# vklyukin/nf_distillation

Hardware: NVIDIA B200
Metric: kd_train_samples_per_sec (higher is better)
Workload: dtype bf16

## Files before the change

nf_distillation_b200/csrc/zpath.cu:

```cuda
#include <cuda_bf16.h>
#include <cuda_runtime.h>
#include <cstdint>

#include "../../include/nfk.h"
#include "launch_util.h"
#include "ptx.cuh"

namespace nfk {

constexpr int ZT = 256;

__device__ __forceinline__ uint32_t bf2(float lo, float hi) {
  __nv_bfloat162 v = __floats2bfloat162_rn(lo, hi);
  return *reinterpret_cast<uint32_t*>(&v);
}

__device__ __forceinline__ void sigmoid_logsigmoid(float t, float& s, float& ls) {
  const float e = expf(-fabsf(t));
  const float l1p = log1pf(e);
  if (t >= 0.f) {
    s = 1.f / (1.f + e);
    ls = -l1p;
  } else {
    s = e / (1.f + e);
    ls = t - l1p;
  }
}

struct Geo {
  int B, HW, W, H;
  int ipc;
  int pixt;
  int og;
  int lgHW, lgW;
};

__device__ __forceinline__ void copy_out_rows(uint4* __restrict__ out4, const uint4* __restrict__ cst, int npix,
                                              int r16, int rs16, int tid) {
  if ((r16 & (r16 - 1)) == 0 && r16 <= ZT) {
    const int lg = __ffs(r16) - 1;
    const int c4 = tid & (r16 - 1), step = ZT >> lg;
    for (int pl = tid >> lg; pl < npix; pl += step) out4[(pl << lg) + c4] = cst[pl * rs16 + c4];
  } else {
    for (int i = tid; i < npix * r16; i += ZT) {
      const int pl = i / r16, c4 = i - pl * r16;
      out4[i] = cst[pl * rs16 + c4];
    }
  }
}

template <int C>
__global__ void __launch_bounds__(ZT)
affine1x1_fwd_kernel(const float* __restrict__ x, const float* __restrict__ Wf, const float* __restrict__ bf,
                     const float* __restrict__ sl, float* __restrict__ y, __nv_bfloat16* __restrict__ col,
                     const float* __restrict__ ld_in, float* __restrict__ ld_out, Geo g, int K1p) {
  pdl_launch_dependents();
  pdl_wait();
  extern __shared__ float sm[];
  constexpr int CH = C / 2;
  float* Ws = sm;
  float* bs = Ws + C * C;
  float* y1s = bs + C;
  float* cst_raw = y1s + ((CH * (g.pixt + 1) + 3) & ~3);
  const int tid = threadIdx.x;
  const int b0 = blockIdx.x * g.ipc;
  const int nimg = min(g.ipc, g.B - b0);
  const int npix = nimg << g.lgHW;
  const int ldp = g.pixt + 1;
  const int HWm = g.HW - 1, Wm = g.W - 1;

  const int pixb = ZT / g.og;
  const int og = tid / pixb;
  const int opg = C / g.og;
  constexpr bool PREFETCH_X = C <= 24;
  float xv[C];
  if (PREFETCH_X) {
    const int pl = tid % pixb;
    if (pl < npix && og < g.og) {
      const float* xp = x + (static_cast<long long>(b0 + (pl >> g.lgHW)) * C << g.lgHW) + (pl & HWm);
#pragma unroll
      for (int i = 0; i < C; ++i) xv[i] = __ldg(xp + (static_cast<long long>(i) << g.lgHW));
    }
  }
  if (Wf) {
    constexpr int W4 = C * C / 4, WPT = (W4 + ZT - 1) / ZT;
    float4 wreg[WPT];
#pragma unroll
    for (int k = 0; k < WPT; ++k) {
      const int i = tid + k * ZT;
      if (i < W4) wreg[k] = __ldg(reinterpret_cast<const float4*>(Wf) + i);
    }
#pragma unroll
    for (int k = 0; k < WPT; ++k) {
      const int i = tid + k * ZT;
      if (i < W4) reinterpret_cast<float4*>(Ws)[i] = wreg[k];
    }
    for (int i = tid; i < C; i += ZT) bs[i] = bf[i];
  }
  if (ld_out && tid < nimg) ld_out[b0 + tid] = ld_in[b0 + tid] + sl[0] * static_cast<float>(g.HW);
  __syncthreads();

  for (int pl = tid % pixb; pl < npix && og < g.og; pl += pixb) {
    const int img = pl >> g.lgHW, p = pl & HWm;
    const float* xp = x + (static_cast<long long>(b0 + img) * C << g.lgHW) + p;
    if (!PREFETCH_X || pl >= pixb) {
#pragma unroll
      for (int i = 0; i < C; ++i) xv[i] = __ldg(xp + (static_cast<long long>(i) << g.lgHW));
    }
    if (Wf) {
      float* yp = y + (static_cast<long long>(b0 + img) * C << g.lgHW) + p;
      for (int o = og * opg; o < (og + 1) * opg; ++o) {
        float acc = bs[o];
        const float4* wr = reinterpret_cast<const float4*>(Ws + o * C);
#pragma unroll
        for (int i = 0; i < C / 4; ++i) {
          const float4 w = wr[i];
          acc = fmaf(w.x, xv[4 * i], acc);
          acc = fmaf(w.y, xv[4 * i + 1], acc);
          acc = fmaf(w.z, xv[4 * i + 2], acc);
          acc = fmaf(w.w, xv[4 * i + 3], acc);
        }
        yp[static_cast<long long>(o) << g.lgHW] = acc;
        if (col && o < CH) y1s[o * ldp + pl] = acc;
      }
    } else if (col) {
#pragma unroll
      for (int o = 0; o < CH; ++o)
        if (o >= og * opg && o < (og + 1) * opg) y1s[o * ldp + pl] = xv[o];
    }
  }
  if (!col) return;
  __syncthreads();
  constexpr int K1 = 9 * CH;
  constexpr int NCH = (K1 + 7) / 8;
  const int r16 = K1p / 8;
  const int rs16 = r16 + 1;
  uint4* cst = reinterpret_cast<uint4*>(cst_raw);
  int noff[9];
#pragma unroll
  for (int tap = 0; tap < 9; ++tap) noff[tap] = (tap / 3 - 1) * g.W + (tap % 3 - 1);
  const int GR = g.pixt >= ZT ? 1 : ZT / g.pixt;
  const int gid = tid / g.pixt;
  for (int pl = GR > 1 ? (tid & (g.pixt - 1)) : tid; pl < npix; pl += (GR > 1 ? g.pixt : ZT)) {
    const int rem = pl & HWm;
    const int yy = rem >> g.lgW, xx = rem & Wm;
    uint32_t vmask = 0;
#pragma unroll
    for (int tap = 0; tap < 9; ++tap) {
      const int ny = yy + tap / 3 - 1, nx = xx + tap % 3 - 1;
      vmask |= (ny >= 0 && ny < g.H && nx >= 0 && nx < g.W) ? (1u << tap) : 0u;
    }
    const float* yb = y1s + pl;
    uint4* drow = cst + pl * rs16;
#pragma unroll
    for (int c4 = 0; c4 < NCH; ++c4) {
      if (GR > 1 && (c4 & (GR - 1)) != gid) continue;
      float v[8];
#pragma unroll
      for (int e = 0; e < 8; ++e) {
        constexpr int dummy = 0; (void)dummy;
        const int k = c4 * 8 + e;
        if (k < K1) {
          const int tap = k / CH, ci = k % CH;
          v[e] = ((vmask >> tap) & 1u) ? yb[ci * ldp + noff[tap]] : 0.f;
        } else {
          v[e] = 0.f;
        }
      }
      drow[c4] = make_uint4(bf2(v[0], v[1]), bf2(v[2], v[3]), bf2(v[4], v[5]), bf2(v[6], v[7]));
    }
    for (int c4 = NCH; c4 < r16; ++c4)
      if (GR == 1 || (c4 & (GR - 1)) == gid) drow[c4] = make_uint4(0u, 0u, 0u, 0u);
  }
  __syncthreads();
  uint4* out4 = reinterpret_cast<uint4*>(col + (static_cast<long long>(b0) << g.lgHW) * K1p);
  copy_out_rows(out4, cst, npix, r16, rs16, tid);
}

template <int C>
__global__ void __launch_bounds__(ZT)
coupling_fwd_kernel(const float* __restrict__ P, int K3p, const float* __restrict__ bias3, float* __restrict__ y,
                    float* __restrict__ hsave, float* __restrict__ ld, Geo g, int reverse) {
  constexpr int J = C / 2;
  const long long M = static_cast<long long>(g.B) << g.lgHW;
  const long long item = static_cast<long long>(blockIdx.x) * ZT + threadIdx.x;
  const long long m = item / J;
  const int j = static_cast<int>(item - m * J);
  const bool live = m < M;
  const int lane = threadIdx.x & 31;
  float lsum = 0.f;
  int b = -1;
  if (live) {
    b = static_cast<int>(m >> g.lgHW);
    const int rem = static_cast<int>(m) & (g.HW - 1);
    const int yy = rem >> g.lgW, xx = rem & (g.W - 1);
    float sh = __ldg(bias3 + 2 * j), lg = __ldg(bias3 + 2 * j + 1);
    const float* prow = P + m * K3p + 2 * j;
#pragma unroll
    for (int tap = 0; tap < 9; ++tap) {
      const int dy = tap / 3 - 1, dx = tap % 3 - 1;
      const int ny = yy + dy, nx = xx + dx;
      if (ny >= 0 && ny < g.H && nx >= 0 && nx < g.W) {
        const float2 v = __ldg(reinterpret_cast<const float2*>(prow + static_cast<long long>(dy * g.W + dx) * K3p +
                                                               tap * C));
        sh += v.x;
        lg += v.y;
      }
    }
    if (hsave) *reinterpret_cast<float2*>(hsave + m * C + 2 * j) = make_float2(sh, lg);
    float s, lsv;
    sigmoid_logsigmoid(lg + 2.f, s, lsv);
    float* yp = y + ((static_cast<long long>(b) * C + J + j) << g.lgHW) + rem;
    const float z2 = *yp;
    *yp = reverse ? (z2 / s - sh) : (z2 + sh) * s;
    lsum = reverse ? -lsv : lsv;
  }
  if (ld) {
#pragma unroll
    for (int o = 1; o < 32; o <<= 1) {
      const float v = __shfl_down_sync(0xffffffffu, lsum, o);
      const int bb = __shfl_down_sync(0xffffffffu, b, o);
      if (lane + o < 32 && bb == b) lsum += v;
    }
    const int bp = __shfl_up_sync(0xffffffffu, b, 1);
    if (live && (lane == 0 || bp != b)) atomicAdd(ld + b, lsum);
  }
}

template <int C>
__global__ void __launch_bounds__(ZT)
coupling_bwd_kernel(const float* __restrict__ g_out, const float* __restrict__ g_ld, const float* __restrict__ z_out,
                    const float* __restrict__ hsave, float* __restrict__ dy, __nv_bfloat16* __restrict__ dhcol,
                    int K3p, float* __restrict__ dbias3, Geo g, int brows) {
  pdl_launch_dependents();
  pdl_wait();
  extern __shared__ float sm[];
  constexpr int J = C / 2;
  const int bands = g.H / brows;
  const bool banded = bands > 1;
  const int halo = banded ? g.W : 0;
  const int tile = banded ? brows * g.W : g.pixt;
  const int ldp = tile + 2 * halo + 1;
  float* dhs = sm;
  float* dbs = dhs + C * ldp;
  uint4* cst = reinterpret_cast<uint4*>(dbs + ((C + 3) & ~3));
  const int tid = threadIdx.x;
  const int HWm = g.HW - 1, Wm = g.W - 1;
  const int ngroups = banded ? g.B * bands : (g.B + g.ipc - 1) / g.ipc;
  constexpr int K3 = 9 * C;
  constexpr int NCH = (K3 + 7) / 8;
  const int r16 = K3p / 8, rs16 = r16 + 1;
  int noff[9];
#pragma unroll
  for (int tap = 0; tap < 9; ++tap) noff[tap] = -((tap / 3 - 1) * g.W + (tap % 3 - 1));
  for (int i = tid; i < C; i += ZT) dbs[i] = 0.f;

  for (int grp = blockIdx.x; grp < ngroups; grp += gridDim.x) {
    const int b0 = banded ? grp / bands : grp * g.ipc;
    const int p0 = banded ? (grp - b0 * bands) * tile : 0;
    const int nimg = banded ? 1 : min(g.ipc, g.B - b0);
    const int npix = banded ? tile : nimg << g.lgHW;
    const int np2 = npix + 2 * halo;
    __syncthreads();
    constexpr int UN = 4;
    for (int i0 = tid; i0 < J * np2; i0 += UN * ZT) {
      float g1[UN], g2[UN], o2[UN], glv[UN];
      float2 hh[UN];
      long long lo[UN];
      int pqv[UN], jjv[UN];
      bool inr[UN], ownv[UN];
#pragma unroll
      for (int u = 0; u < UN; ++u) {
        const int i = i0 + u * ZT;
        const int jj = i / np2, pq = i - jj * np2;
        const int pl = pq - halo;
        const int img = banded ? 0 : pl >> g.lgHW;
        const int rem = banded ? p0 + pl : pl & HWm;
        jjv[u] = jj; pqv[u] = pq;
        ownv[u] = i < J * np2 && pl >= 0 && pl < npix;
        inr[u] = i < J * np2 && rem >= 0 && rem < g.HW;
        g1[u] = g2[u] = o2[u] = glv[u] = 0.f;
        hh[u] = make_float2(0.f, 0.f);
        lo[u] = 0;
        if (inr[u]) {
          lo[u] = ((static_cast<long long>(b0 + img) * C + jj) << g.lgHW) + rem;
          const long long hi = lo[u] + (static_cast<long long>(J) << g.lgHW);
          const long long m = (static_cast<long long>(b0 + img) << g.lgHW) + rem;
          g2[u] = g_out[hi];
          o2[u] = z_out[hi];
          hh[u] = *reinterpret_cast<const float2*>(hsave + m * C + 2 * jj);
          glv[u] = g_ld[b0 + img];
          if (ownv[u]) g1[u] = g_out[lo[u]];
        }
      }
#pragma unroll
      for (int u = 0; u < UN; ++u) {
        if (i0 + u * ZT >= J * np2) continue;
        float dsh = 0.f, dlg = 0.f;
        if (inr[u]) {
          float sg, lsv;
          sigmoid_logsigmoid(hh[u].y + 2.f, sg, lsv);
          dsh = g2[u] * sg;
          dlg = (g2[u] * o2[u] + glv[u]) * (1.f - sg);
          if (ownv[u]) {
            dy[lo[u]] = g1[u];
            dy[lo[u] + (static_cast<long long>(J) << g.lgHW)] = dsh;
          }
        }
        const int jj = jjv[u];
        dhs[(2 * jj) * ldp + pqv[u]] = dsh;
        dhs[(2 * jj + 1) * ldp + pqv[u]] = dlg;
        float a = ownv[u] ? dsh : 0.f, bsum = ownv[u] ? dlg : 0.f;
        if ((np2 & 31) == 0) {
          for (int o = 16; o > 0; o >>= 1) {
            a += __shfl_xor_sync(0xffffffffu, a, o);
            bsum += __shfl_xor_sync(0xffffffffu, bsum, o);
          }
          if ((tid & 31) == 0) { atomicAdd(&dbs[2 * jj], a); atomicAdd(&dbs[2 * jj + 1], bsum); }
        } else {
          atomicAdd(&dbs[2 * jj], a);
          atomicAdd(&dbs[2 * jj + 1], bsum);
        }
      }
    }
    __syncthreads();
    const int GR = tile >= ZT ? 1 : ZT / tile;
    const int gid = tid / tile;
    for (int pl = GR > 1 ? (tid & (tile - 1)) : tid; pl < npix; pl += (GR > 1 ? tile : ZT)) {
      const int rem = banded ? p0 + pl : pl & HWm;
      const int yy = rem >> g.lgW, xx = rem & Wm;
      uint32_t vmask = 0;
#pragma unroll
      for (int tap = 0; tap < 9; ++tap) {
        const int ny = yy - (tap / 3 - 1), nx = xx - (tap % 3 - 1);
        vmask |= (ny >= 0 && ny < g.H && nx >= 0 && nx < g.W) ? (1u << tap) : 0u;
      }
      const float* db = dhs + halo + pl;
      uint4* drow = cst + pl * rs16;
#pragma unroll
      for (int c4 = 0; c4 < NCH; ++c4) {
        if (GR > 1 && (c4 & (GR - 1)) != gid) continue;
        float v[8];
#pragma unroll
        for (int e = 0; e < 8; ++e) {
          const int k = c4 * 8 + e;
          if (k < K3) {
            const int tap = k / C, co = k % C;
            v[e] = ((vmask >> tap) & 1u) ? db[co * ldp + noff[tap]] : 0.f;
          } else {
            v[e] = 0.f;
          }
        }
        drow[c4] = make_uint4(bf2(v[0], v[1]), bf2(v[2], v[3]), bf2(v[4], v[5]), bf2(v[6], v[7]));
      }
      for (int c4 = NCH; c4 < r16; ++c4)
        if (GR == 1 || (c4 & (GR - 1)) == gid) drow[c4] = make_uint4(0u, 0u, 0u, 0u);
    }
    __syncthreads();
    uint4* out4 = reinterpret_cast<uint4*>(dhcol + ((static_cast<long long>(b0) << g.lgHW) + p0) * K3p);
    copy_out_rows(out4, cst, npix, r16, rs16, tid);
  }
  __syncthreads();
  for (int i = tid; i < C; i += ZT) atomicAdd(dbias3 + i, dbs[i]);
}

template <int C>
__global__ void __launch_bounds__(ZT)
affine1x1_bwd_kernel(const float* __restrict__ dy, const float* __restrict__ dcol, int K1p,
                     const float* __restrict__ x, const float* __restrict__ Wf, float* __restrict__ dx,
                     float* __restrict__ dWf, float* __restrict__ dbf, Geo g, int tile_floats) {
  pdl_launch_dependents();
  pdl_wait();
  extern __shared__ float sm[];
  constexpr int CH = C / 2;
  const int ldp = g.pixt + 1;
  float* WT = sm;
  float* dys = WT + C * C;
  float* xs = dys + C * ldp;
  float* acc = dys + tile_floats;
  const int tid = threadIdx.x;
  const int HWm = g.HW - 1, Wm = g.W - 1;
  const int ngroups = (g.B + g.ipc - 1) / g.ipc;

  for (int i = tid; i < C * C; i += ZT) {
    const int o = i / C, c = i % C;
    WT[c * C + o] = Wf[i];
  }
  for (int i = tid; i < C * C + C; i += ZT) acc[i] = 0.f;
  constexpr int NBK = (C / 4) * (C / 4);
  constexpr int SL = NBK >= ZT ? 1 : ZT / NBK;
  constexpr int RB = (NBK + ZT - 1) / ZT;
  float wacc[RB][4][4] = {};

  for (int grp = blockIdx.x; grp < ngroups; grp += gridDim.x) {
    const int b0 = grp * g.ipc;
    const int nimg = min(g.ipc, g.B - b0);
    const int npix = nimg << g.lgHW;
    __syncthreads();
    {
      constexpr int UL = 4;
      const int total = C * npix;
      for (int i0 = tid; i0 < total; i0 += UL * ZT) {
        float xv[UL], dv[UL];
        int so[UL];
#pragma unroll
        for (int u = 0; u < UL; ++u) {
          const int i = i0 + u * ZT;
          xv[u] = dv[u] = 0.f;
          so[u] = -1;
          if (i < total) {
            const int c = i / npix, pl = i - c * npix;
            const int img = pl >> g.lgHW, rem = pl & HWm;
            const long long gi = ((static_cast<long long>(b0 + img) * C + c) << g.lgHW) + rem;
            xv[u] = x[gi];
            dv[u] = dy[gi];
            so[u] = c * ldp + pl;
          }
        }
#pragma unroll
        for (int u = 0; u < UL; ++u)
          if (so[u] >= 0) { xs[so[u]] = xv[u]; dys[so[u]] = dv[u]; }
      }
    }
    __syncthreads();
    if (dcol) {
      constexpr int UN = 3;
      for (int i0 = tid; i0 < CH * npix; i0 += UN * ZT) {
        float v[UN][9];
#pragma unroll
        for (int u = 0; u < UN; ++u) {
          const int i = i0 + u * ZT;
          const bool live = i < CH * npix;
          const int pl = live ? i / CH : 0, ci = live ? i - pl * CH : 0;
          const int rem = pl & HWm;
          const int yy = rem >> g.lgW, xx = rem & Wm;
          const long long m = (static_cast<long long>(b0) << g.lgHW) + pl;
#pragma unroll
          for (int tap = 0; tap < 9; ++tap) {
            const int ddy = tap / 3 - 1, ddx = tap % 3 - 1;
            const int ny = yy - ddy, nx = xx - ddx;
            v[u][tap] = (live && ny >= 0 && ny < g.H && nx >= 0 && nx < g.W)
                            ? __ldg(dcol + (m - ddy * g.W - ddx) * K1p + tap * CH + ci) : 0.f;
          }
        }
#pragma unroll
        for (int u = 0; u < UN; ++u) {
          const int i = i0 + u * ZT;
          if (i < CH * npix) {
            const int pl = i / CH, ci = i - pl * CH;
            float a = 0.f;
#pragma unroll
            for (int tap = 0; tap < 9; ++tap) a += v[u][tap];
            dys[ci * ldp + pl] += a;
          }
        }
      }
      __syncthreads();
    }
    for (int pl = tid; pl < npix; pl += ZT) {
      const int img = pl >> g.lgHW, rem = pl & HWm;
      float dv[C];
#pragma unroll
      for (int o = 0; o < C; ++o) dv[o] = dys[o * ldp + pl];
      float* dxp = dx + ((static_cast<long long>(b0 + img) * C) << g.lgHW) + rem;
#pragma unroll 4
      for (int i = 0; i < C; ++i) {
        float a = 0.f;
        const float4* wr = reinterpret_cast<const float4*>(WT + i * C);
#pragma unroll
        for (int o = 0; o < C / 4; ++o) {
          const float4 w = wr[o];
          a = fmaf(w.x, dv[4 * o], a);
          a = fmaf(w.y, dv[4 * o + 1], a);
          a = fmaf(w.z, dv[4 * o + 2], a);
          a = fmaf(w.w, dv[4 * o + 3], a);
        }
        dxp[static_cast<long long>(i) << g.lgHW] = a;
      }
    }
#pragma unroll
    for (int rb = 0; rb < RB; ++rb) {
      const int blk = (NBK < ZT ? tid % NBK : tid) + rb * ZT;
      const int slice = NBK < ZT ? tid / NBK : 0;
      if (blk >= NBK || slice >= SL) continue;
      const int to = blk / (C / 4), ti = blk % (C / 4);
      for (int p = slice; p < npix; p += SL) {
        float dv[4], xv[4];
#pragma unroll
        for (int q = 0; q < 4; ++q) {
          dv[q] = dys[(4 * to + q) * ldp + p];
          xv[q] = xs[(4 * ti + q) * ldp + p];
        }
#pragma unroll
        for (int q = 0; q < 4; ++q)
#pragma unroll
          for (int r = 0; r < 4; ++r) wacc[rb][q][r] = fmaf(dv[q], xv[r], wacc[rb][q][r]);
      }
    }
    {
      const int warp = tid >> 5, lane = tid & 31;
      for (int o = warp; o < C; o += ZT / 32) {
        float a = 0.f;
        for (int p = lane; p < npix; p += 32) a += dys[o * ldp + p];
        for (int sft = 16; sft > 0; sft >>= 1) a += __shfl_xor_sync(0xffffffffu, a, sft);
        if (lane == 0) acc[C * C + o] += a;
      }
    }
  }
  __syncthreads();
  float* scratch = dys;
#pragma unroll
  for (int rb = 0; rb < RB; ++rb) {
    const int blk = (NBK < ZT ? tid % NBK : tid) + rb * ZT;
    const int slice = NBK < ZT ? tid / NBK : 0;
    if (blk >= NBK || slice >= SL) continue;
    const int to = blk / (C / 4), ti = blk % (C / 4);
#pragma unroll
    for (int q = 0; q < 4; ++q)
#pragma unroll
      for (int r = 0; r < 4; ++r) scratch[slice * C * C + (4 * to + q) * C + 4 * ti + r] = wacc[rb][q][r];
  }
  __syncthreads();
  for (int i = tid; i < C * C; i += ZT) {
    float a = 0.f;
    for (int sl2 = 0; sl2 < SL; ++sl2) a += scratch[sl2 * C * C + i];
    acc[i] += a;
  }
  __syncthreads();
  for (int i = tid; i < C * C; i += ZT) atomicAdd(dWf + i, acc[i]);
  for (int i = tid; i < C; i += ZT) atomicAdd(dbf + i, acc[C * C + i]);
}

static Geo make_geo(int B, int C, int H, int W, bool heavy) {
  Geo g;
  g.B = B; g.H = H; g.W = W; g.HW = H * W;
  int target = heavy ? (C <= 24 ? 256 : (C <= 48 ? 128 : 64)) : 256;
  g.ipc = g.HW >= target ? 1 : target / g.HW;
  if (g.ipc > B) g.ipc = B;
  while (g.ipc > 1 && (B + g.ipc - 1) / g.ipc < 2 * 148) g.ipc >>= 1;
  g.pixt = g.ipc * g.HW;
  g.og = 1;
  g.lgW = 0; while ((1 << g.lgW) < W) ++g.lgW;
  g.lgHW = 0; while ((1 << g.lgHW) < g.HW) ++g.lgHW;
  return g;
}

static bool pow2(int v) { return v > 0 && (v & (v - 1)) == 0; }

template <typename K>
static int ensure_smem(K kernel, int bytes) {
  return ensure_dyn_smem(reinterpret_cast<const void*>(kernel), bytes);
}

#define NFK_DISPATCH_C(C_, ...)                             \
  switch (C_) {                                             \
    case 12: { constexpr int CC = 12; __VA_ARGS__; } break; \
    case 24: { constexpr int CC = 24; __VA_ARGS__; } break; \
    case 48: { constexpr int CC = 48; __VA_ARGS__; } break; \
    case 96: { constexpr int CC = 96; __VA_ARGS__; } break; \
    default: return NFK_ERR_SHAPE;                          \
  }

}

using namespace nfk;

extern "C" int nfk_affine1x1_fwd(const float* x, const float* Wf, const float* bf, const float* sl, float* y,
                                 void* col, int K1p, const float* ld_in, float* ld_out, int B, int C, int H, int W,
                                 void* stream) {
  if (B <= 0 || H <= 0 || W <= 0 || H * W > 4096 || !pow2(H) || !pow2(W)) return NFK_ERR_SHAPE;
  if (!x || (!Wf && !col) || (Wf && (!bf || !y)) || (ld_out && (!ld_in || !sl))) return NFK_ERR_ARG;
  if (col && (K1p % 64 || K1p < 9 * (C / 2))) return NFK_ERR_SHAPE;
  Geo g = make_geo(B, C, H, W, false);
  if (col) {
    while (g.ipc > 1 && static_cast<long long>(g.pixt) * (K1p * 2 + 16) > 64 * 1024) { g.ipc >>= 1; g.pixt = g.ipc * g.HW; }
  }
  {
    const long long M = static_cast<long long>(B) * H * W;
    g.og = M >= 131072 ? 1 : (M >= 32768 ? 2 : (M >= 8192 && C < 48 ? 4 : 8));
    while (g.og > 1 && (C % g.og || (C / g.og) % 2)) g.og >>= 1;
  }
  if (col && g.HW <= 16)
    while (g.pixt < 128 && 2 * g.ipc <= B && (B + 2 * g.ipc - 1) / (2 * g.ipc) >= 148) { g.ipc <<= 1; g.pixt = g.ipc * g.HW; }
  const int smem = (C * C + C + (col ? (C / 2) * (g.pixt + 1) + 4 + g.pixt * (K1p / 8 + 1) * 4 : 0)) * 4;
  const int grid = (B + g.ipc - 1) / g.ipc;
  cudaStream_t st = static_cast<cudaStream_t>(stream);
  NFK_DISPATCH_C(C, {
    int rc = ensure_smem(affine1x1_fwd_kernel<CC>, smem);
    if (rc) return rc;
    if (launch_pdl(affine1x1_fwd_kernel<CC>, dim3(grid), dim3(ZT), smem, st, x, Wf, bf, sl, y,
                   static_cast<__nv_bfloat16*>(col), ld_in, ld_out, g, K1p) != cudaSuccess)
      return NFK_ERR_LAUNCH;
  });
  return cudaGetLastError() == cudaSuccess ? NFK_OK : NFK_ERR_LAUNCH;
}

extern "C" int nfk_coupling_fwd(const float* P, int K3p, const float* bias3, float* y, float* hsave, float* ld,
                                int B, int C, int H, int W, int reverse, void* stream) {
  if (B <= 0 || H <= 0 || W <= 0 || H * W > 4096 || K3p < 9 * C || K3p % 2 || !pow2(H) || !pow2(W))
    return NFK_ERR_SHAPE;
  if (!P || !bias3 || !y) return NFK_ERR_ARG;
  Geo g = make_geo(B, C, H, W, false);
  const long long items = static_cast<long long>(B) * H * W * (C / 2);
  const unsigned grid = static_cast<unsigned>((items + ZT - 1) / ZT);
  cudaStream_t st = static_cast<cudaStream_t>(stream);
  NFK_DISPATCH_C(C, { coupling_fwd_kernel<CC><<<grid, ZT, 0, st>>>(P, K3p, bias3, y, hsave, ld, g, reverse); });
  return cudaGetLastError() == cudaSuccess ? NFK_OK : NFK_ERR_LAUNCH;
}

extern "C" int nfk_coupling_bwd(const float* g_out, const float* g_ld, const float* z_out, const float* hsave,
                                float* dy, void* dhcol, int K3p, float* dbias3, int B, int C, int H, int W,
                                void* stream) {
  if (B <= 0 || H <= 0 || W <= 0 || H * W > 4096 || K3p % 64 || K3p < 9 * C || !pow2(H) || !pow2(W))
    return NFK_ERR_SHAPE;
  if (!g_out || !g_ld || !z_out || !hsave || !dy || !dhcol || !dbias3) return NFK_ERR_ARG;
  Geo g = make_geo(B, C, H, W, true);
  auto bytes = [&](int tile, int halo) {
    return static_cast<long long>(C * (tile + 2 * halo + 1) + ((C + 3) & ~3)) * 4 +
           static_cast<long long>(tile) * (K3p / 8 + 1) * 16 + 16;
  };
  while (g.ipc > 1 && bytes(g.pixt, 0) > 100 * 1024) { g.ipc >>= 1; g.pixt = g.ipc * g.HW; }
  int brows = H;
  if (g.ipc == 1)
    while (brows > 1 && bytes(brows * W, brows < H ? W : 0) > 100 * 1024) brows >>= 1;
  const bool banded = brows < H;
  const int smem = static_cast<int>(bytes(banded ? brows * W : g.pixt, banded ? W : 0));
  const int groups = banded ? B * (H / brows) : (B + g.ipc - 1) / g.ipc;
  const int grid = groups < 4 * 148 ? groups : 4 * 148;
  cudaStream_t st = static_cast<cudaStream_t>(stream);
  NFK_DISPATCH_C(C, {
    int rc = ensure_smem(coupling_bwd_kernel<CC>, smem);
    if (rc) return rc;
    if (launch_pdl(coupling_bwd_kernel<CC>, dim3(grid), dim3(ZT), smem, st, g_out, g_ld, z_out, hsave, dy,
                   static_cast<__nv_bfloat16*>(dhcol), K3p, dbias3, g, brows) != cudaSuccess)
      return NFK_ERR_LAUNCH;
  });
  return cudaGetLastError() == cudaSuccess ? NFK_OK : NFK_ERR_LAUNCH;
}

extern "C" int nfk_affine1x1_bwd(const float* dy, const float* dcol, int K1p, const float* x, const float* Wf,
                                 float* dx, float* dWf, float* dbf, int B, int C, int H, int W, void* stream) {
  if (B <= 0 || H <= 0 || W <= 0 || H * W > 4096 || !pow2(H) || !pow2(W)) return NFK_ERR_SHAPE;
  if (!dy || !x || !Wf || !dx || !dWf || !dbf) return NFK_ERR_ARG;
  Geo g = make_geo(B, C, H, W, true);
  const int nbk = (C / 4) * (C / 4);
  const int slices = nbk >= ZT ? 1 : ZT / nbk;
  int tile_floats = 2 * C * (g.pixt + 1);
  if (tile_floats < slices * C * C) tile_floats = slices * C * C;
  const int smem = (C * C + tile_floats + C * C + C) * 4;
  const int groups = (B + g.ipc - 1) / g.ipc;
  const int grid = groups < 4 * 148 ? groups : 4 * 148;
  cudaStream_t st = static_cast<cudaStream_t>(stream);
  NFK_DISPATCH_C(C, {
    int rc = ensure_smem(affine1x1_bwd_kernel<CC>, smem);
    if (rc) return rc;
    if (launch_pdl(affine1x1_bwd_kernel<CC>, dim3(grid), dim3(ZT), smem, st, dy, dcol, K1p, x, Wf, dx, dWf, dbf, g,
                   tile_floats) != cudaSuccess)
      return NFK_ERR_LAUNCH;
  });
  return cudaGetLastError() == cudaSuccess ? NFK_OK : NFK_ERR_LAUNCH;
}
```

Measured before the change: 54280.

## Pipeline affine 1x1 backward with TMA bulk loads into double-buffered smem ring

Rewrites the invertible 1x1 affine backward kernel to prefetch x, dy and the dcol halo tiles into a two-stage shared-memory ring. The loads use cp.async.bulk and TMA 2D loads with 128B swizzle, completed through mbarriers, so the next group's data arrives while the current group is computed. It also sizes threads per block by channel count, adds row-band tiling for large images, splits output channels across thread groups, and picks grid size from an occupancy query. The cost is much more shared memory and complexity, plus the risk of swizzle or indexing bugs and lower occupancy.

```diff
diff --git a/nf_distillation_b200/csrc/zpath.cu b/nf_distillation_b200/csrc/zpath.cu
--- a/nf_distillation_b200/csrc/zpath.cu
+++ b/nf_distillation_b200/csrc/zpath.cu
@@ -1,6 +1,8 @@
+#include <cuda.h>
 #include <cuda_bf16.h>
 #include <cuda_runtime.h>
 #include <cstdint>
+#include <cstring>
 
 #include "../../include/nfk.h"
 #include "launch_util.h"
@@ -364,124 +366,185 @@
   for (int i = tid; i < C; i += ZT) atomicAdd(dbias3 + i, dbs[i]);
 }
 
+struct AbwdArgs {
+  const float *dy, *x, *Wf;
+  float *dx, *dWf, *dbf;
+  int B, H, W, lgHW, lgW;
+  int U, lgU;
+  int ipc;
+  int bands;
+  int ngroups;
+  int R, nbox, RT;
+  int xoff_dy, xoff_dcol, stage_floats;
+  int ldp;
+  int og;
+  int has_dcol;
+};
+
+__device__ __forceinline__ void bulk_g2s(float* dst, const float* src, uint32_t bytes, uint64_t* bar) {
+  asm volatile("cp.async.bulk.shared::cluster.global.mbarrier::complete_tx::bytes [%0], [%1], %2, [%3];"
+               ::"r"(smem_u32(dst)), "l"(src), "r"(bytes), "r"(smem_u32(bar))
+               : "memory");
+}
+__device__ __forceinline__ void bulk_g2s_elect(float* dst, const float* src, uint32_t bytes, uint64_t* bar) {
+  asm volatile(
+      "{\n\t.reg .pred q;\n\t"
+      "elect.sync _|q, 0xffffffff;\n\t"
+      "@q cp.async.bulk.shared::cluster.global.mbarrier::complete_tx::bytes [%0], [%1], %2, [%3];\n\t}\n"
+      ::"r"(smem_u32(dst)), "l"(src), "r"(bytes), "r"(smem_u32(bar))
+      : "memory");
+}
+
+__host__ __device__ constexpr int abwd_threads(int C) { return C <= 12 ? 1024 : (C <= 48 ? 512 : 256); }
+
 template <int C>
-__global__ void __launch_bounds__(ZT)
-affine1x1_bwd_kernel(const float* __restrict__ dy, const float* __restrict__ dcol, int K1p,
-                     const float* __restrict__ x, const float* __restrict__ Wf, float* __restrict__ dx,
-                     float* __restrict__ dWf, float* __restrict__ dbf, Geo g, int tile_floats) {
+__global__ void __launch_bounds__(abwd_threads(C))
+affine1x1_bwd_kernel(const __grid_constant__ CUtensorMap tmD, const AbwdArgs a) {
+  constexpr int NT = abwd_threads(C);
   pdl_launch_dependents();
+  extern __shared__ unsigned char sm_raw[];
+  constexpr int CH = C / 2, K1 = 9 * CH, NSLAB = (K1 + 31) / 32;
+  float* ring = reinterpret_cast<float*>(sm_raw + ((1024u - (smem_u32(sm_raw) & 1023u)) & 1023u));
+  float* WT = ring + 2 * a.stage_floats;
+  float* xs = WT + C * C;
+  float* dys = xs + C * a.ldp;
+  float* acc = dys + C * a.ldp;
+  uint64_t* full = reinterpret_cast<uint64_t*>(acc + C * C + C);
+  const int tid = threadIdx.x, warp = tid >> 5;
+  const int HW = 1 << a.lgHW, HWm = HW - 1, Wm = a.W - 1, Um = a.U - 1;
+  const bool banded = a.bands > 1;
+  const int halo = banded ? a.W : 0;
+  if (tid == 0) {
+    mbar_init(&full[0], 1);
+    mbar_init(&full[1], 1);
+    fence_mbar_init();
+  }
+  if (warp == 0 && a.has_dcol) tma_prefetch_desc(&tmD);
+  __syncthreads();
   pdl_wait();
-  extern __shared__ float sm[];
-  constexpr int CH = C / 2;
-  const int ldp = g.pixt + 1;
-  float* WT = sm;
-  float* dys = WT + C * C;
-  float* xs = dys + C * ldp;
-  float* acc = dys + tile_floats;
-  const int tid = threadIdx.x;
-  const int HWm = g.HW - 1, Wm = g.W - 1;
-  const int ngroups = (g.B + g.ipc - 1) / g.ipc;
-
-  for (int i = tid; i < C * C; i += ZT) {
+
+  auto issue = [&](int grp, int s) {
+    float* st = ring + s * a.stage_floats;
+    const int b0 = banded ? grp / a.bands : grp * a.ipc;
+    const int p0 = banded ? (grp - b0 * a.bands) * a.U : 0;
+    const int nimg = banded ? 1 : min(a.ipc, a.B - b0);
+    const uint32_t xbytes = static_cast<uint32_t>(nimg * C * a.U) * 4u;
+    const uint32_t dbytes = a.has_dcol ? static_cast<uint32_t>(NSLAB * a.RT) * 128u : 0u;
+    mbar_expect_tx_elect(&full[s], 2u * xbytes + dbytes);
+    __syncwarp();
+    if (banded) {
+      const int lane = tid & 31;
+      for (int c = lane; c < C; c += 32) {
+        const long long go = ((static_cast<long long>(b0) * C + c) << a.lgHW) + p0;
+        bulk_g2s(st + c * a.U, a.x + go, xbytes / C, &full[s]);
+        bulk_g2s(st + a.xoff_dy + c * a.U, a.dy + go, xbytes / C, &full[s]);
+      }
+    } else {
+      const long long go = (static_cast<long long>(b0) * C) << a.lgHW;
+      bulk_g2s_elect(st, a.x + go, xbytes, &full[s]);
+      bulk_g2s_elect(st + a.xoff_dy, a.dy + go, xbytes, &full[s]);
+    }
+    if (a.has_dcol) {
+      const int m0 = (b0 << a.lgHW) + p0 - halo;
+#pragma unroll 1
+      for (int j = 0; j < NSLAB; ++j)
+#pragma unroll 1
+        for (int k = 0; k < a.nbox; ++k)
+          tma_load_2d_elect(st + a.xoff_dcol + (j * a.RT + k * a.R) * 32, &tmD, &full[s], j * 32, m0 + k * a.R);
+    }
+  };
+  if (warp == 0)
+    for (int s = 0; s < 2; ++s) {
+      const int grp = blockIdx.x + s * gridDim.x;
+      if (grp < a.ngroups) issue(grp, s);
+    }
+
+  for (int i = tid; i < C * C; i += NT) {
     const int o = i / C, c = i % C;
-    WT[c * C + o] = Wf[i];
-  }
-  for (int i = tid; i < C * C + C; i += ZT) acc[i] = 0.f;
+    WT[c * C + o] = a.Wf[i];
+  }
+  for (int i = tid; i < C * C + C; i += NT) acc[i] = 0.f;
   constexpr int NBK = (C / 4) * (C / 4);
-  constexpr int SL = NBK >= ZT ? 1 : ZT / NBK;
-  constexpr int RB = (NBK + ZT - 1) / ZT;
+  constexpr int SL = NBK >= NT ? 1 : NT / NBK;
+  constexpr int RB = (NBK + NT - 1) / NT;
   float wacc[RB][4][4] = {};
-
-  for (int grp = blockIdx.x; grp < ngroups; grp += gridDim.x) {
-    const int b0 = grp * g.ipc;
-    const int nimg = min(g.ipc, g.B - b0);
-    const int npix = nimg << g.lgHW;
+  const int ldp = a.ldp;
+
+  int it = 0;
+  for (int grp = blockIdx.x; grp < a.ngroups; grp += gridDim.x, ++it) {
+    const int s = it & 1;
+    const float* st = ring + s * a.stage_floats;
+    const int b0 = banded ? grp / a.bands : grp * a.ipc;
+    const int p0 = banded ? (grp - b0 * a.bands) * a.U : 0;
+    const int nimg = banded ? 1 : min(a.ipc, a.B - b0);
+    const int npix = nimg * a.U;
     __syncthreads();
+    mbar_wait(&full[s], (it >> 1) & 1);
     {
-      constexpr int UL = 4;
-      const int total = C * npix;
-      for (int i0 = tid; i0 < total; i0 += UL * ZT) {
-        float xv[UL], dv[UL];
-        int so[UL];
-#pragma unroll
-        for (int u = 0; u < UL; ++u) {
-          const int i = i0 + u * ZT;
-          xv[u] = dv[u] = 0.f;
-          so[u] = -1;
-          if (i < total) {
-            const int c = i / npix, pl = i - c * npix;
-            const int img = pl >> g.lgHW, rem = pl & HWm;
-            const long long gi = ((static_cast<long long>(b0 + img) * C + c) << g.lgHW) + rem;
-            xv[u] = x[gi];
-            dv[u] = dy[gi];
-            so[u] = c * ldp + pl;
+      const int cu = C * a.U;
+      for (int unit = 0; unit < nimg; ++unit)
+        for (int r = tid; r < cu; r += NT) {
+          const int c = r >> a.lgU, pl = unit * a.U + (r & Um), i = unit * cu + r;
+          xs[c * ldp + pl] = st[i];
+          if (!a.has_dcol || c >= CH) dys[c * ldp + pl] = st[a.xoff_dy + i];
+        }
+    }
+    if (a.has_dcol) {
+      const float* ds = st + a.xoff_dcol;
+      for (int i = tid; i < CH * npix; i += NT) {
+        const int pl = i / CH, ci = i - pl * CH;
+        const int rem = banded ? p0 + pl : pl & HWm;
+        const int yy = rem >> a.lgW, xx = rem & Wm;
+        const int r0 = halo + pl;
+        float acc9 = 0.f;
+#pragma unroll
+        for (int tap = 0; tap < 9; ++tap) {
+          const int ddy = tap / 3 - 1, ddx = tap % 3 - 1;
+          const int ny = yy - ddy, nx = xx - ddx;
+          float v = 0.f;
+          if (ny >= 0 && ny < a.H && nx >= 0 && nx < a.W) {
+            const int r = r0 - ddy * a.W - ddx, c = tap * CH + ci;
+            v = ds[((c >> 5) * a.RT + r) * 32 + ((((c >> 2) & 7) ^ (r & 7)) << 2) + (c & 3)];
           }
-        }
-#pragma unroll
-        for (int u = 0; u < UL; ++u)
-          if (so[u] >= 0) { xs[so[u]] = xv[u]; dys[so[u]] = dv[u]; }
+          acc9 += v;
+        }
+        const int sidx = (((pl >> a.lgU) * C + ci) << a.lgU) + (pl & Um);
+        dys[ci * ldp + pl] = st[a.xoff_dy + sidx] + acc9;
       }
     }
     __syncthreads();
-    if (dcol) {
-      constexpr int UN = 3;
-      for (int i0 = tid; i0 < CH * npix; i0 += UN * ZT) {
-        float v[UN][9];
-#pragma unroll
-        for (int u = 0; u < UN; ++u) {
-          const int i = i0 + u * ZT;
-          const bool live = i < CH * npix;
-          const int pl = live ? i / CH : 0, ci = live ? i - pl * CH : 0;
-          const int rem = pl & HWm;
-          const int yy = rem >> g.lgW, xx = rem & Wm;
-          const long long m = (static_cast<long long>(b0) << g.lgHW) + pl;
-#pragma unroll
-          for (int tap = 0; tap < 9; ++tap) {
-            const int ddy = tap / 3 - 1, ddx = tap % 3 - 1;
-            const int ny = yy - ddy, nx = xx - ddx;
-            v[u][tap] = (live && ny >= 0 && ny < g.H && nx >= 0 && nx < g.W)
-                            ? __ldg(dcol + (m - ddy * g.W - ddx) * K1p + tap * CH + ci) : 0.f;
+    if (warp == 0) {
+      const int nxt = grp + 2 * gridDim.x;
+      if (nxt < a.ngroups) issue(nxt, s);
+    }
+    {
+      const int pixb = NT / a.og, ogi = tid / pixb, opg = C / a.og;
+      for (int pl = tid - ogi * pixb; pl < npix && ogi < a.og; pl += pixb) {
+        const int unit = pl >> a.lgU, u = pl & Um;
+        float dv[C];
+#pragma unroll
+        for (int o = 0; o < C; ++o) dv[o] = dys[o * ldp + pl];
+        float* dxp = a.dx + ((static_cast<long long>(banded ? b0 : b0 + unit) * C) << a.lgHW) + p0 + u;
+#pragma unroll 4
+        for (int i = ogi * opg; i < (ogi + 1) * opg; ++i) {
+          float acc1 = 0.f;
+          const float4* wr = reinterpret_cast<const float4*>(WT + i * C);
+#pragma unroll
+          for (int o = 0; o < C / 4; ++o) {
+            const float4 w = wr[o];
+            acc1 = fmaf(w.x, dv[4 * o], acc1);
+            acc1 = fmaf(w.y, dv[4 * o + 1], acc1);
+            acc1 = fmaf(w.z, dv[4 * o + 2], acc1);
+            acc1 = fmaf(w.w, dv[4 * o + 3], acc1);
           }
-        }
-#pragma unroll
-        for (int u = 0; u < UN; ++u) {
-          const int i = i0 + u * ZT;
-          if (i < CH * npix) {
-            const int pl = i / CH, ci = i - pl * CH;
-            float a = 0.f;
-#pragma unroll
-            for (int tap = 0; tap < 9; ++tap) a += v[u][tap];
-            dys[ci * ldp + pl] += a;
-          }
-        }
-      }
-      __syncthreads();
-    }
-    for (int pl = tid; pl < npix; pl += ZT) {
-      const int img = pl >> g.lgHW, rem = pl & HWm;
-      float dv[C];
-#pragma unroll
-      for (int o = 0; o < C; ++o) dv[o] = dys[o * ldp + pl];
-      float* dxp = dx + ((static_cast<long long>(b0 + img) * C) << g.lgHW) + rem;
-#pragma unroll 4
-      for (int i = 0; i < C; ++i) {
-        float a = 0.f;
-        const float4* wr = reinterpret_cast<const float4*>(WT + i * C);
-#pragma unroll
-        for (int o = 0; o < C / 4; ++o) {
-          const float4 w = wr[o];
-          a = fmaf(w.x, dv[4 * o], a);
-          a = fmaf(w.y, dv[4 * o + 1], a);
-          a = fmaf(w.z, dv[4 * o + 2], a);
-          a = fmaf(w.w, dv[4 * o + 3], a);
-        }
-        dxp[static_cast<long long>(i) << g.lgHW] = a;
+          dxp[static_cast<long long>(i) << a.lgHW] = acc1;
+        }
       }
     }
 #pragma unroll
     for (int rb = 0; rb < RB; ++rb) {
-      const int blk = (NBK < ZT ? tid % NBK : tid) + rb * ZT;
-      const int slice = NBK < ZT ? tid / NBK : 0;
+      const int blk = (NBK < NT ? tid % NBK : tid) + rb * NT;
+      const int slice = NBK < NT ? tid / NBK : 0;
       if (blk >= NBK || slice >= SL) continue;
       const int to = blk / (C / 4), ti = blk % (C / 4);
       for (int p = slice; p < npix; p += SL) {
@@ -498,21 +561,21 @@
       }
     }
     {
-      const int warp = tid >> 5, lane = tid & 31;
-      for (int o = warp; o < C; o += ZT / 32) {
-        float a = 0.f;
-        for (int p = lane; p < npix; p += 32) a += dys[o * ldp + p];
-        for (int sft = 16; sft > 0; sft >>= 1) a += __shfl_xor_sync(0xffffffffu, a, sft);
-        if (lane == 0) acc[C * C + o] += a;
+      const int lane = tid & 31;
+      for (int o = warp; o < C; o += NT / 32) {
+        float s1 = 0.f;
+        for (int p = lane; p < npix; p += 32) s1 += dys[o * ldp + p];
+        for (int sft = 16; sft > 0; sft >>= 1) s1 += __shfl_xor_sync(0xffffffffu, s1, sft);
+        if (lane == 0) acc[C * C + o] += s1;
       }
     }
   }
   __syncthreads();
-  float* scratch = dys;
+  float* scratch = ring;
 #pragma unroll
   for (int rb = 0; rb < RB; ++rb) {
-    const int blk = (NBK < ZT ? tid % NBK : tid) + rb * ZT;
-    const int slice = NBK < ZT ? tid / NBK : 0;
+    const int blk = (NBK < NT ? tid % NBK : tid) + rb * NT;
+    const int slice = NBK < NT ? tid / NBK : 0;
     if (blk >= NBK || slice >= SL) continue;
     const int to = blk / (C / 4), ti = blk % (C / 4);
 #pragma unroll
@@ -521,14 +584,14 @@
       for (int r = 0; r < 4; ++r) scratch[slice * C * C + (4 * to + q) * C + 4 * ti + r] = wacc[rb][q][r];
   }
   __syncthreads();
-  for (int i = tid; i < C * C; i += ZT) {
-    float a = 0.f;
-    for (int sl2 = 0; sl2 < SL; ++sl2) a += scratch[sl2 * C * C + i];
-    acc[i] += a;
+  for (int i = tid; i < C * C; i += NT) {
+    float s1 = 0.f;
+    for (int sl2 = 0; sl2 < SL; ++sl2) s1 += scratch[sl2 * C * C + i];
+    acc[i] += s1;
   }
   __syncthreads();
-  for (int i = tid; i < C * C; i += ZT) atomicAdd(dWf + i, acc[i]);
-  for (int i = tid; i < C; i += ZT) atomicAdd(dbf + i, acc[C * C + i]);
+  for (int i = tid; i < C * C; i += NT) atomicAdd(a.dWf + i, acc[i]);
+  for (int i = tid; i < C; i += NT) atomicAdd(a.dbf + i, acc[C * C + i]);
 }
 
 static Geo make_geo(int B, int C, int H, int W, bool heavy) {
@@ -550,6 +613,44 @@
 template <typename K>
 static int ensure_smem(K kernel, int bytes) {
   return ensure_dyn_smem(reinterpret_cast<const void*>(kernel), bytes);
+}
+
+typedef CUresult (*EncodeTiledFnZ)(CUtensorMap*, CUtensorMapDataType, cuuint32_t, void*, const cuuint64_t*,
+                                   const cuuint64_t*, const cuuint32_t*, const cuuint32_t*, CUtensorMapInterleave,
+                                   CUtensorMapSwizzle, CUtensorMapL2promotion, CUtensorMapFloatOOBfill);
+
+static int zp_tmap_f32(CUtensorMap* m, const void* ptr, uint64_t cols, uint64_t rows, uint64_t ld, uint32_t box_rows) {
+  static EncodeTiledFnZ fn = nullptr;
+  if (!fn) {
+    void* p = nullptr;
+    cudaDriverEntryPointQueryResult q;
+    if (cudaGetDriverEntryPoint("cuTensorMapEncodeTiled", &p, cudaEnableDefault, &q) != cudaSuccess ||
+        q != cudaDriverEntryPointSuccess)
+      return NFK_ERR_DRIVER;
+    fn = reinterpret_cast<EncodeTiledFnZ>(p);
+  }
+  if ((reinterpret_cast<uintptr_t>(ptr) & 15) || (ld * 4) % 16) return NFK_ERR_ALIGN;
+  cuuint64_t dims[2] = {cols, rows};
+  cuuint64_t strides[1] = {ld * 4};
+  cuuint32_t box[2] = {32, box_rows};
+  cuuint32_t estr[2] = {1, 1};
+  CUresult r = fn(m, CU_TENSOR_MAP_DATA_TYPE_FLOAT32, 2, const_cast<void*>(ptr), dims, strides, box, estr,
+                  CU_TENSOR_MAP_INTERLEAVE_NONE, CU_TENSOR_MAP_SWIZZLE_128B, CU_TENSOR_MAP_L2_PROMOTION_L2_256B,
+                  CU_TENSOR_MAP_FLOAT_OOB_FILL_NONE);
+  return r == CUDA_SUCCESS ? NFK_OK : NFK_ERR_DRIVER;
+}
+
+static int occupancy(const void* kernel, int threads, int smem) {
+  static std::mutex mu;
+  static std::unordered_map<unsigned long long, int> memo;
+  const unsigned long long key = (reinterpret_cast<uintptr_t>(kernel) << 20) ^ static_cast<unsigned>(smem);
+  std::lock_guard<std::mutex> lock(mu);
+  auto it = memo.find(key);
+  if (it != memo.end()) return it->second;
+  int n = 1;
+  if (cudaOccupancyMaxActiveBlocksPerMultiprocessor(&n, kernel, threads, smem) != cudaSuccess || n < 1) n = 1;
+  memo[key] = n;
+  return n;
 }
 
 #define NFK_DISPATCH_C(C_, ...)                             \
@@ -642,20 +743,74 @@
                                  float* dx, float* dWf, float* dbf, int B, int C, int H, int W, void* stream) {
   if (B <= 0 || H <= 0 || W <= 0 || H * W > 4096 || !pow2(H) || !pow2(W)) return NFK_ERR_SHAPE;
   if (!dy || !x || !Wf || !dx || !dWf || !dbf) return NFK_ERR_ARG;
-  Geo g = make_geo(B, C, H, W, true);
-  const int nbk = (C / 4) * (C / 4);
-  const int slices = nbk >= ZT ? 1 : ZT / nbk;
-  int tile_floats = 2 * C * (g.pixt + 1);
-  if (tile_floats < slices * C * C) tile_floats = slices * C * C;
-  const int smem = (C * C + tile_floats + C * C + C) * 4;
-  const int groups = (B + g.ipc - 1) / g.ipc;
-  const int grid = groups < 4 * 148 ? groups : 4 * 148;
+  if (C != 12 && C != 24 && C != 48 && C != 96) return NFK_ERR_SHAPE;
+  const int CH = C / 2, K1 = 9 * CH, nslab = (K1 + 31) / 32;
+  if (dcol && K1p < K1) return NFK_ERR_SHAPE;
+  if ((reinterpret_cast<uintptr_t>(x) | reinterpret_cast<uintptr_t>(dy)) & 15) return NFK_ERR_ALIGN;
+  const int HW = H * W;
+  AbwdArgs a{};
+  a.dy = dy; a.x = x; a.Wf = Wf; a.dx = dx; a.dWf = dWf; a.dbf = dbf;
+  a.B = B; a.H = H; a.W = W;
+  a.lgW = 0; while ((1 << a.lgW) < W) ++a.lgW;
+  a.lgHW = 0; while ((1 << a.lgHW) < HW) ++a.lgHW;
+  a.has_dcol = dcol != nullptr;
+  int dev = 0, sms = 148;
+  cudaGetDevice(&dev);
+  cudaDeviceGetAttribute(&sms, cudaDevAttrMultiProcessorCount, dev);
+  const int nt = abwd_threads(C);
+  const int nbk = (C / 4) * (C / 4), slices = nbk >= nt ? 1 : nt / nbk;
+  auto plan = [&](int units, int U, int rows) {
+    a.ipc = units; a.U = U;
+    a.R = rows < 256 ? (rows + 7) & ~7 : 256;
+    a.nbox = (rows + a.R - 1) / a.R;
+    a.RT = a.nbox * a.R;
+    a.xoff_dy = units * C * U;
+    a.xoff_dcol = (2 * units * C * U + 255) & ~255;
+    a.stage_floats = a.has_dcol ? a.xoff_dcol + nslab * a.RT * 32 : a.xoff_dcol;
+    a.ldp = units * U + 1;
+    long long ringf = 2LL * a.stage_floats;
+    if (ringf < static_cast<long long>(slices) * C * C) ringf = static_cast<long long>(slices) * C * C;
+    a.stage_floats = static_cast<int>((ringf / 2 + 255) & ~255LL);
+    return 1024 + (2LL * a.stage_floats + 2LL * C * C + 2LL * C * a.ldp + C) * 4 + 16;
+  };
+  constexpr long long kStage = 96 * 1024, kSmem = 227 * 1024;
+  auto stage_bytes = [&]() { return static_cast<long long>(a.stage_floats) * 4; };
+  int ipc = (B + 4 * sms - 1) / (4 * sms);
+  long long smem = 0;
+  a.bands = 1;
+  for (; ipc >= 1; --ipc) {
+    smem = plan(ipc, HW, ipc * HW);
+    if (stage_bytes() <= kStage && smem <= kSmem) break;
+  }
+  if (ipc < 1) {
+    int brows = H / 2;
+    for (; brows >= 1; brows >>= 1) {
+      if ((brows * W) % 4) { brows = 0; break; }
+      smem = plan(1, brows * W, brows * W + 2 * W);
+      if (stage_bytes() <= kStage && smem <= kSmem) break;
+    }
+    if (brows < 1) return NFK_ERR_SHAPE;
+    a.bands = H / brows;
+  }
+  a.lgU = 0; while ((1 << a.lgU) < a.U) ++a.lgU;
+  a.ngroups = a.bands > 1 ? B * a.bands : (B + a.ipc - 1) / a.ipc;
+  const int npmax = a.ipc * a.U;
+  a.og = 1;
+  while (2 * a.og * npmax <= nt && C % (2 * a.og) == 0) a.og *= 2;
+  CUtensorMap tmD;
+  memset(&tmD, 0, sizeof(tmD));
+  if (dcol) {
+    const int rc = zp_tmap_f32(&tmD, dcol, K1, static_cast<uint64_t>(B) * HW, K1p, a.R);
+    if (rc) return rc;
+  }
   cudaStream_t st = static_cast<cudaStream_t>(stream);
   NFK_DISPATCH_C(C, {
-    int rc = ensure_smem(affine1x1_bwd_kernel<CC>, smem);
+    int rc = ensure_smem(affine1x1_bwd_kernel<CC>, static_cast<int>(smem));
     if (rc) return rc;
-    if (launch_pdl(affine1x1_bwd_kernel<CC>, dim3(grid), dim3(ZT), smem, st, dy, dcol, K1p, x, Wf, dx, dWf, dbf, g,
-                   tile_floats) != cudaSuccess)
+    const int per_sm = occupancy(reinterpret_cast<const void*>(affine1x1_bwd_kernel<CC>), nt, static_cast<int>(smem));
+    const int grid = a.ngroups < per_sm * sms ? a.ngroups : per_sm * sms;
+    if (launch_pdl(affine1x1_bwd_kernel<CC>, dim3(grid), dim3(nt), static_cast<size_t>(smem), st, tmD, a) !=
+        cudaSuccess)
       return NFK_ERR_LAUNCH;
   });
   return cudaGetLastError() == cudaSuccess ? NFK_OK : NFK_ERR_LAUNCH;
```

Result: no change. 54550, median of 6 (+0.5%).
